# rusty-fast-solvers/rusty-compression

Measured on AMD Instinct MI355X. Metric: GB/s + compressions/sec, 8192x8192 f64 rank-128 rSVD+ID, higher is better.
Workload: dtype f64

## Files before the change

rusty_compression_amd/csrc/kernels_tsqr.hip:

```cpp
#include "rc_common.hpp"
#include "rc_device.hpp"

namespace rc {

static __host__ __device__ inline int64_t cdiv(int64_t a, int64_t b) { return (a + b - 1) / b; }

template <typename T> struct TNum;
template <> struct TNum<double> {
    static __device__ inline double tol3z() { return 1.0536712127723509e-08; }
    static __device__ inline double tiny() { return 1e-300; }
};
template <> struct TNum<float> {
    static __device__ inline float tol3z() { return 2.44140625e-04f; }
    static __device__ inline float tiny() { return 1e-30f; }
};

template <typename T>
__device__ inline T wave_sum64(T v) {
#pragma unroll
    for (int off = 32; off > 0; off >>= 1) v += __shfl_xor(v, off, 64);
    return v;
}
template <typename T>
__device__ inline T row_sum16(T v) {
#pragma unroll
    for (int off = 8; off > 0; off >>= 1) v += __shfl_xor(v, off, 64);
    return v;
}

template <typename T, int NT>
__global__ __launch_bounds__(1024) void k_chol_inv(Mat<T> g, Mat<T> r_out, Mat<T> rinv_out, int check_identity, T ident_tol, T skip_tol, int *flag) {
    extern __shared__ __attribute__((aligned(16))) char smem_raw[];
    const int n = (int)g.rows;
    const int ld = n | 1;
    T *A = reinterpret_cast<T *>(smem_raw);
    T *svec = A + (size_t)n * ld;
    T *rowbuf = svec + n;
    T *red = rowbuf + 2 * n;
    const int tid = threadIdx.x, lane = tid & 63, wv = tid >> 6;
    const int ti = tid >> 5, tc = tid & 31;

    T reg[NT][NT];
    T dev = 0;
#pragma unroll
    for (int a = 0; a < NT; ++a)
#pragma unroll
        for (int b = 0; b < NT; ++b) {
            const int i = ti + 32 * a, c = tc + 32 * b;
            T v = 0;
            if (i < n && c < n) {
                v = g.at(i, c);
                dev = max(dev, fabs(v - ((i == c) ? (T)1 : (T)0)));
            }
            reg[a][b] = v;
// ... 74 lines not shown
                }
            } else if (i > j && i < n) {
                const T w = rb[i] * invd;
#pragma unroll
                for (int b = a; b < NT; ++b) reg[a][b] -= w * cv[b];
            }
            if (i <= j) {
                const T xj = cb[i];
                const T w = xj * invd;
#pragma unroll
                for (int b = a; b < NT; ++b) {
                    xr[a][b] -= w * cv[b];
                    if (b == ja && tc == jt) xr[a][b] = xj * invr;
                }
            }
        }
    }
#pragma unroll
    for (int a = 0; a < NT; ++a)
#pragma unroll
        for (int b = 0; b < NT; ++b) {
            const int i = ti + 32 * a, c = tc + 32 * b;
            if (i < n && c < n) {
                r_out.at(i, c) = (b >= a && c >= i) ? reg[a][b] : (T)0;
                rinv_out.at(i, c) = (b >= a && c >= i) ? xr[a][b] : (T)0;
            }
        }
}

template <typename T>
static size_t chol_lds(int64_t n) { return ((size_t)n * (n | 1) + 3 * (size_t)n + 16) * sizeof(T); }

template <typename T, int NT>
static void chol_inv_launch(rc_context *c, Mat<T> g, Mat<T> r, Mat<T> rinv, bool check_identity, T ident_tol, T skip_tol, int *flag) {
    auto kern = k_chol_inv<T, NT>;
    static bool attr_set[64] = {};
    if (!attr_set[c->device & 63]) {
        RC_HIP(hipFuncSetAttribute(reinterpret_cast<const void *>(kern), hipFuncAttributeMaxDynamicSharedMemorySize, 160 * 1024 - 1024));
        attr_set[c->device & 63] = true;
    }
    hipLaunchKernelGGL(kern, dim3(1), dim3(1024), chol_lds<T>(g.rows), c->stream, g, r, rinv, check_identity ? 1 : 0, ident_tol, skip_tol, flag);
}
template <typename T>
static void chol_inv(rc_context *c, Mat<T> g, Mat<T> r, Mat<T> rinv, bool check_identity, T ident_tol, T skip_tol, int *flag) {
    const int64_t n = g.rows;
    RC_REQUIRE(n <= 224 && chol_lds<T>(n) <= 160 * 1024 - 1024, RC_INVALID_ARGUMENT, "chol_inv: n = %lld does not fit LDS", (long long)n);
    ProfScope ps(c, "op:chol_inv n=%lld", (long long)n);
    if (n <= 64) chol_inv_launch<T, 2>(c, g, r, rinv, check_identity, ident_tol, skip_tol, flag);
    else if (n <= 160) chol_inv_launch<T, 5>(c, g, r, rinv, check_identity, ident_tol, skip_tol, flag);
    else chol_inv_launch<T, 7>(c, g, r, rinv, check_identity, ident_tol, skip_tol, flag);
}

template <typename T>
bool tsqr_supported(int64_t m, int64_t n) {
    const size_t small_lds = ((size_t)n * (n | 1) + 4 * (size_t)n) * sizeof(T) + (size_t)n * sizeof(int) + 256;
    return n >= 2 && m >= 4 * n && m >= 1024 && small_lds <= 160 * 1024 - 2048;
}

template <typename T>
void tsqr_cholqr2_factored(rc_context *c, Mat<T> y, Mat<T> q1, Mat<T> r2i, Mat<T> r, int *flag) {
    const int64_t m = y.rows, n = y.cols;
    ProfScope ps(c, "op:cholqr2 %lldx%lld", (long long)m, (long long)n);
    ArenaMark mark(c);
    Mat<T> g = rowmajor(c->alloc<T>((size_t)n * even_ld(n)), n, n, even_ld(n));
    Mat<T> r1 = rowmajor(c->alloc<T>((size_t)n * even_ld(n)), n, n, even_ld(n)), r1i = rowmajor(c->alloc<T>((size_t)n * even_ld(n)), n, n, even_ld(n));
    Mat<T> r2 = rowmajor(c->alloc<T>((size_t)n * even_ld(n)), n, n, even_ld(n));
    gemm<T>(c, 1, y.t(), y, 0, g);
    chol_inv<T>(c, g, r1, r1i, false, 0, 0, flag);
    gemm<T>(c, 1, y, r1i, 0, q1);
    gemm<T>(c, 1, q1.t(), q1, 0, g);
    static const int skip_ok = [] { const char *e = getenv("RC_CHOLQR_SKIP"); return e ? atoi(e) : 1; }();
    const T skip_tol = skip_ok ? (sizeof(T) == 8 ? (T)2.5e-14 : (T)1e-6) : (T)-1;
    chol_inv<T>(c, g, r2, r2i, true, (T)1e-2, skip_tol, flag);
    gemm<T>(c, 1, r2, r1, 0, r);
}

template <typename T>
void tsqr_cholqr2(rc_context *c, Mat<T> y, Mat<T> q, Mat<T> r, int *flag) {
    const int64_t m = y.rows, n = y.cols;
    ArenaMark mark(c);
    Mat<T> q1 = rowmajor(c->alloc<T>((size_t)m * even_ld(n)), m, n, even_ld(n));
    Mat<T> r2i = rowmajor(c->alloc<T>((size_t)n * even_ld(n)), n, n, even_ld(n));
    tsqr_cholqr2_factored<T>(c, y, q1, r2i, r, flag);
    gemm<T>(c, 1, q1, r2i, 0, q);
}

template <typename T>
__device__ inline T safe_hypot(T a, T b) {
    a = fabs(a); b = fabs(b);
    const T w = max(a, b), z = min(a, b);
    if (z == (T)0) return w;
    const T q = z * fast_rcp(w);
    const T e = (T)1 + q * q;
    return w * (e * fast_rsqrt(e));
}
template <typename T>
__device__ inline T fast_sqrt_pos(T x) { return x > (T)0 ? x * fast_rsqrt(x) : (T)0; }

template <typename T, int NEJ, int LPP>
__device__ __forceinline__ void qrcp_small_apply(T *A, int ld, int n, int j, int grp, int ll, int ngrp, const int *jp, T *vn1, T *vn2, T tj, int pivot, bool safe) {
    const T *vcol = A + jp[j] * ld;
    T v[NEJ];
#pragma unroll
    for (int e = 0; e < NEJ; ++e) {
        int i = j + ll + LPP * e;
        v[e] = (i < n) ? ((i == j) ? (T)1 : vcol[i]) : (T)0;
    }
    for (int p = j + 1 + grp; p < n; p += ngrp) {
        T *xcol = A + jp[p] * ld;
        T x[NEJ];
        T dot = 0;
        if (safe) {
#pragma unroll
            for (int e = 0; e < NEJ; ++e) {
                x[e] = xcol[j + ll + LPP * e];
                dot = fma(v[e], x[e], dot);
            }
        } else {
#pragma unroll
            for (int e = 0; e < NEJ; ++e) {
                int i = j + ll + LPP * e;
                x[e] = (i < n) ? xcol[i] : (T)0;
                dot = fma(v[e], x[e], dot);
            }
        }
        if (tj != (T)0) {
            dot = group_sum_dpp<LPP>(dot);
            const T f = tj * dot;
#pragma unroll
            for (int e = 0; e < NEJ; ++e) {
                int i = j + ll + LPP * e;
                if (i < n) { x[e] -= f * v[e]; xcol[i] = x[e]; }
            }
        }
        if (pivot) {
            const T xj = xcol[j];
            const T vn = vn1[p];
            if (vn != (T)0) {
                T t = fabs(xj) * fast_rcp(vn);
                T temp = (T)1 - t * t;
                temp = temp > (T)0 ? temp : (T)0;
                T rr = vn * fast_rcp(vn2[p]);
                T temp2 = temp * rr * rr;
                if (temp2 <= TNum<T>::tol3z()) {
                    T ss = 0;
#pragma unroll
                    for (int e = 0; e < NEJ; ++e) {
                        int i = j + ll + LPP * e;
                        if (i > j && i < n) ss += x[e] * x[e];
                    }
                    ss = group_sum_dpp<LPP>(ss);
                    if (ll == 0) { T nn = (j < n - 1) ? fast_sqrt_pos(ss) : (T)0; vn1[p] = nn; vn2[p] = nn; }
                } else if (ll == 0) {
                    vn1[p] = vn * fast_sqrt_pos(temp);
                }
            }
        }
    }
}

template <typename T, int NE, int LPP, int E0>
__device__ __forceinline__ void qrcp_small_reflect(T (&x)[NE], const T *vcol, T tj, int j, int n, int ll) {
    T v[NE];
    T dot = 0;
#pragma unroll
    for (int e = E0; e < NE; ++e) {
        int i = ll + LPP * e;
        v[e] = 0;
        if (i < n && i >= j) { v[e] = (i == j) ? (T)1 : vcol[i]; dot = fma(v[e], x[e], dot); }
    }
    dot = group_sum_dpp<LPP>(dot);
    const T f = tj * dot;
#pragma unroll
    for (int e = E0; e < NE; ++e) x[e] -= f * v[e];
}

template <typename T, int NE, int NTHR>
__global__ __launch_bounds__(NTHR) void k_qrcp_small(Mat<T> rin, int kmax, int pivot, int64_t *jpvt_out, Mat<T> rout, Mat<T> q2) {
    constexpr int LPP = 8;
    constexpr int NGRP = NTHR / LPP;
    extern __shared__ __attribute__((aligned(16))) char smem_raw[];
    const int n = (int)rin.rows;
    const int ld = n | 1;
    T *A = reinterpret_cast<T *>(smem_raw);
    T *vn1 = A + (size_t)n * ld;
    T *vn2 = vn1 + n;
    T *tau = vn2 + n;
    int *jp = reinterpret_cast<int *>(tau + n);
    const int tid = threadIdx.x, lane = tid & 63;
    const int ll = tid % LPP, grp = tid / LPP;
    const bool safe = LPP * NE <= 3 * n;

    for (int e = tid; e < n * n; e += NTHR) {
        int i = e % n, cc = e / n;
        A[cc * ld + i] = rin.at(i, cc);
    }
    __syncthreads();
    for (int p = grp; p < n; p += NGRP) {
        T acc = 0;
        for (int i = ll; i < n; i += LPP) { T v = A[p * ld + i]; acc += v * v; }
        acc = group_sum_dpp<LPP>(acc);
        if (ll == 0) { T nr = sqrt(acc); vn1[p] = nr; vn2[p] = nr; jp[p] = p; tau[p] = (T)0; }
    }
    __syncthreads();

    for (int j = 0; j < kmax; ++j) {
        if (tid < 64) {
            if (pivot) {
                T best = (T)-1;
                int bi = 0x7fffffff;
                for (int p = j + lane; p < n; p += 64) {
                    T v = fabs(vn1[p]);
                    if (v > best) { best = v; bi = p; }
                }
                const T mx = wave_max_dpp(best);
                const int pv = wave_min_dpp(best == mx ? bi : 0x7fffffff);
                const int pvt = (pv >= j && pv < n) ? pv : j;
                if (lane == 0 && pvt != j) {
                    int t = jp[pvt]; jp[pvt] = jp[j]; jp[j] = t;
                    vn1[pvt] = vn1[j];
                    vn2[pvt] = vn2[j];
                }
                __builtin_amdgcn_fence(__ATOMIC_ACQ_REL, "wavefront");
            }
            T *col = A + jp[j] * ld;
            const T alpha = col[j];
            T acc = 0;
            for (int i = j + 1 + lane; i < n; i += 64) { T v = col[i]; acc += v * v; }
            acc = wave_sum_dpp(acc);
            const T xnorm = fast_sqrt_pos(acc);
            if (xnorm == (T)0) {
                if (lane == 0) tau[j] = 0;
            } else {
                const T beta = -copysign(safe_hypot(alpha, xnorm), alpha);
                const T scal = fast_rcp(alpha - beta);
                for (int i = j + 1 + lane; i < n; i += 64) col[i] *= scal;
                if (lane == 0) { tau[j] = (beta - alpha) * fast_rcp(beta); col[j] = beta; }
            }
        }
        __syncthreads();
        {
            const int rem = n - j;
            const T tj = tau[j];
            if (NE > 12 && rem > 8 * 12) qrcp_small_apply<T, NE, LPP>(A, ld, n, j, grp, ll, NGRP, jp, vn1, vn2, tj, pivot, safe);
            else if (NE > 8 && rem > 8 * 8) qrcp_small_apply<T, (NE > 12 ? 12 : NE), LPP>(A, ld, n, j, grp, ll, NGRP, jp, vn1, vn2, tj, pivot, safe);
            else if (NE > 4 && rem > 8 * 4) qrcp_small_apply<T, (NE > 8 ? 8 : NE), LPP>(A, ld, n, j, grp, ll, NGRP, jp, vn1, vn2, tj, pivot, safe);
            else qrcp_small_apply<T, (NE > 4 ? 4 : NE), LPP>(A, ld, n, j, grp, ll, NGRP, jp, vn1, vn2, tj, pivot, safe);
        }
        __syncthreads();
    }

    for (int p = tid; p < n; p += NTHR) jpvt_out[p] = jp[p];
    if (!rout.empty()) {
        const int64_t total = rout.rows * rout.cols;
        for (int64_t e = tid; e < total; e += NTHR) {
            int i = (int)(e / rout.cols), p = (int)(e % rout.cols);
            rout.at(i, p) = (i <= p) ? A[jp[p] * ld + i] : (T)0;
        }
    }
    if (!q2.empty()) {
        for (int cq = grp; cq < (int)q2.cols; cq += NGRP) {
            T x[NE];
#pragma unroll
            for (int e = 0; e < NE; ++e) x[e] = (ll + LPP * e == cq) ? (T)1 : (T)0;
            for (int j = (cq < kmax - 1 ? cq : kmax - 1); j >= 0; --j) {
                const T tj = tau[j];
                if (tj == (T)0) continue;
                const T *vcol = A + jp[j] * ld;
                const int e0 = j / LPP;
                if (NE > 12 && e0 >= 12) qrcp_small_reflect<T, NE, LPP, (NE > 12 ? 12 : 0)>(x, vcol, tj, j, n, ll);
                else if (NE > 8 && e0 >= 8) qrcp_small_reflect<T, NE, LPP, (NE > 8 ? 8 : 0)>(x, vcol, tj, j, n, ll);
                else if (NE > 4 && e0 >= 4) qrcp_small_reflect<T, NE, LPP, (NE > 4 ? 4 : 0)>(x, vcol, tj, j, n, ll);
                else qrcp_small_reflect<T, NE, LPP, 0>(x, vcol, tj, j, n, ll);
            }
#pragma unroll
            for (int e = 0; e < NE; ++e) {
                int i = ll + LPP * e;
                if (i < n) q2.at(i, cq) = x[e];
            }
        }
    }
}

template <typename T>
void qrcp_small(rc_context *c, Mat<T> rin, int64_t kmax, bool pivot, int64_t *jpvt, Mat<T> rout, Mat<T> q2) {
    const int64_t n = rin.rows;
    RC_REQUIRE(rin.rows == rin.cols, RC_INVALID_ARGUMENT, "qrcp_small: square input required");
    const size_t lds = ((size_t)n * (n | 1) + 3 * (size_t)n) * sizeof(T) + (size_t)n * sizeof(int) + 64;
    RC_REQUIRE(lds <= 160 * 1024 - 1024 && n <= 208, RC_INVALID_ARGUMENT, "qrcp_small: n = %lld does not fit LDS", (long long)n);
    ProfScope ps(c, "op:qrcp_small n=%lld k=%lld", (long long)n, (long long)kmax);
#define RC_QS(NE, NT_)                                                                                                 \
    do {                                                                                                               \
        auto kern = k_qrcp_small<T, NE, NT_>;                                                                          \
        static bool attr_set[64] = {};                                                                                 \
        if (!attr_set[c->device & 63]) {                                                                               \
            RC_HIP(hipFuncSetAttribute(reinterpret_cast<const void *>(kern), hipFuncAttributeMaxDynamicSharedMemorySize, 160 * 1024 - 1024)); \
            attr_set[c->device & 63] = true;                                                                           \
        }                                                                                                              \
        hipLaunchKernelGGL(kern, dim3(1), dim3(NT_), lds, c->stream, rin, (int)kmax, pivot ? 1 : 0, jpvt, rout, q2);   \
    } while (0)
    static const int wide = [] { const char *e = getenv("RC_QRCP_SMALL_1024"); return e ? atoi(e) : 1; }();
    if (n <= 64) RC_QS(8, 512);
    else if (n <= 144 && wide) RC_QS(18, 1024);
    else if (n <= 144) RC_QS(18, 512);
    else RC_QS(26, 512);
#undef RC_QS
}

template <typename T>
__global__ __launch_bounds__(1024) void k_householder_signs(Mat<T> q, T *d) {
    extern __shared__ __attribute__((aligned(16))) char smem_raw[];
    const int k = (int)q.cols;
    const int ld = k | 1;
    T *W = reinterpret_cast<T *>(smem_raw);
    const int tid = threadIdx.x;
    for (int e = tid; e < k * k; e += 1024) {
        int i = e % k, cc = e / k;
        W[i * ld + cc] = q.at(i, cc);
    }
    __syncthreads();
    const int ti = tid >> 5, tc = tid & 31;
    for (int j = 0; j < k; ++j) {
        const T s = W[j * ld + j];
        const T dj = (s > (T)0) ? (T)-1 : (T)1;
        const T u = (T)1 + fabs(s);
        if (tid == 0) d[j] = dj;
        const T inv = -dj / u;
        for (int i = j + 1 + ti; i < k; i += 32) {
            const T li = W[i * ld + j] * inv;
            for (int cc = j + 1 + tc; cc < k; cc += 32) W[i * ld + cc] -= li * W[j * ld + cc];
        }
        __syncthreads();
    }
}
template <typename T>
__global__ __launch_bounds__(256) void k_scale_cols_rows(Mat<T> q, Mat<T> r, const T *d) {
    const int64_t tq = q.rows * q.cols, tr = r.rows * r.cols;
    for (int64_t e = blockIdx.x * (int64_t)blockDim.x + threadIdx.x; e < tq + tr; e += (int64_t)gridDim.x * blockDim.x) {
        if (e < tq) {
            int64_t j = e / q.rows, i = e - j * q.rows;
            if (d[j] < (T)0) q.at(i, j) = -q.at(i, j);
        } else {
            int64_t f = e - tq;
            int64_t i = f / r.cols, p = f - i * r.cols;
            if (d[i] < (T)0) r.at(i, p) = -r.at(i, p);
        }
    }
}

template <typename T>
static void householder_signs(rc_context *c, Mat<T> top, T *d) {
    const int64_t k = top.cols;
    const size_t lds = (size_t)k * (k | 1) * sizeof(T);
    RC_REQUIRE(top.rows >= k && lds <= 160 * 1024 - 1024, RC_INVALID_ARGUMENT, "sign fix: k = %lld does not fit LDS", (long long)k);
    auto kern = k_householder_signs<T>;
    static bool attr_set[64] = {};
    if (!attr_set[c->device & 63]) {
        RC_HIP(hipFuncSetAttribute(reinterpret_cast<const void *>(kern), hipFuncAttributeMaxDynamicSharedMemorySize, 160 * 1024 - 1024));
        attr_set[c->device & 63] = true;
    }
    hipLaunchKernelGGL(kern, dim3(1), dim3(1024), lds, c->stream, top, d);
}
template <typename T>
static void scale_cols_rows(rc_context *c, Mat<T> q, Mat<T> r, const T *d) {
    const int64_t total = q.rows * q.cols + r.rows * r.cols;
    hipLaunchKernelGGL(k_scale_cols_rows<T>, dim3((unsigned)std::min<int64_t>(cdiv(total, 256), 4096)), dim3(256), 0, c->stream, q, r, d);
}

template <typename T>
void householder_sign_fix(rc_context *c, Mat<T> q, Mat<T> r) {
    const int64_t k = q.cols;
    if (k == 0) return;
    RC_REQUIRE(q.rows >= k, RC_INVALID_ARGUMENT, "sign fix: q must be tall");
    ProfScope ps(c, "op:householder_sign_fix k=%lld", (long long)k);
    ArenaMark mark(c);
    T *d = c->alloc<T>((size_t)k);
    householder_signs<T>(c, q, d);
    scale_cols_rows<T>(c, q, r, d);
}

template <typename T>
void qrcp_tall_fast(rc_context *c, Mat<T> y, int64_t k, bool pivot, Mat<T> q, Mat<T> r, int64_t *ind, int *flag) {
    const int64_t m = y.rows, n = y.cols;
    ProfScope ps(c, "op:qrcp_tall_fast %lldx%lld k=%lld pivot=%d", (long long)m, (long long)n, (long long)k, pivot ? 1 : 0);
    ArenaMark mark(c);
    static const int fold = [] { const char *e = getenv("RC_TSQR_FOLD"); return e ? atoi(e) : 1; }();
    Mat<T> q1 = rowmajor(c->alloc<T>((size_t)m * even_ld(n)), m, n, even_ld(n));
    Mat<T> r1 = colmajor(c->alloc<T>((size_t)n * even_ld(n)), n, n, even_ld(n));
    Mat<T> r2i = rowmajor(c->alloc<T>((size_t)n * even_ld(n)), n, n, even_ld(n));
    if (fold) tsqr_cholqr2_factored<T>(c, y, q1, r2i, r1, flag);
    else tsqr_cholqr2<T>(c, y, q1, r1, flag);
    Mat<T> q2 = colmajor(c->alloc<T>((size_t)even_ld(n) * k), n, k, even_ld(n));
    Mat<T> rr = r.empty() ? rowmajor(c->alloc<T>((size_t)k * even_ld(n)), k, n, even_ld(n)) : r;
    qrcp_small<T>(c, r1, k, pivot, ind, rr, q2);
    Mat<T> qq = q.empty() ? rowmajor(c->alloc<T>((size_t)m * even_ld(k)), m, k, even_ld(k)) : q;
    if (!fold) {
        gemm<T>(c, 1, q1, q2, 0, qq);
        householder_sign_fix<T>(c, qq, rr);
        return;
    }
    Mat<T> w = colmajor(c->alloc<T>((size_t)even_ld(n) * k), n, k, even_ld(n));
    Mat<T> top = colmajor(c->alloc<T>((size_t)even_ld(k) * k), k, k, even_ld(k));
    T *d = c->alloc<T>((size_t)k);
    gemm<T>(c, 1, r2i, q2, 0, w);
    gemm<T>(c, 1, q1.sub(0, k, 0, n), w, 0, top);
    householder_signs<T>(c, top, d);
    scale_cols_rows<T>(c, w, rr, d);
    gemm<T>(c, 1, q1, w, 0, qq);
}

#define RC_INST(T)                                                                                               \
    template bool tsqr_supported<T>(int64_t, int64_t);                                                           \
    template void tsqr_cholqr2<T>(rc_context *, Mat<T>, Mat<T>, Mat<T>, int *);                                  \
    template void tsqr_cholqr2_factored<T>(rc_context *, Mat<T>, Mat<T>, Mat<T>, Mat<T>, int *);                 \
    template void qrcp_small<T>(rc_context *, Mat<T>, int64_t, bool, int64_t *, Mat<T>, Mat<T>);                 \
    template void householder_sign_fix<T>(rc_context *, Mat<T>, Mat<T>);                                         \
    template void qrcp_tall_fast<T>(rc_context *, Mat<T>, int64_t, bool, Mat<T>, Mat<T>, int64_t *, int *);
RC_INST(double)
RC_INST(float)
#undef RC_INST

}
```

rusty_compression_amd/csrc/rc_api.hip:

```cpp
#include "rc_common.hpp"

#include <unistd.h>

#include <atomic>
#include <chrono>

#include <algorithm>
#include <cmath>

using namespace rc;

static constexpr size_t kAlign = 256;

void rc_context::retire_arena() {
    if (arena) {
        if (live_graphs > 0) retired.push_back(arena);
        else (void)hipFree(arena);
    }
    arena = nullptr;
    arena_size = 0;
}

void rc_context::swap_arena() {
    std::swap(arena, aux_arena.base);
// ... 201 lines not shown
    RC_HIP(hipMemcpyAsync(c->pinned, dev, bytes, hipMemcpyDeviceToHost, c->stream));
    RC_HIP(hipStreamSynchronize(c->stream));
    std::memcpy(host, c->pinned, bytes);
}

template <typename T>
Mat<T> tmp_colmajor(rc_context *c, int64_t rows, int64_t cols) {
    int64_t ld = even_ld(std::max<int64_t>(rows, 1));
    return colmajor(c->alloc<T>((size_t)ld * std::max<int64_t>(cols, 1)), rows, cols, ld);
}
template <typename T>
Mat<T> tmp_rowmajor(rc_context *c, int64_t rows, int64_t cols) {
    int64_t ld = even_ld(std::max<int64_t>(cols, 1));
    return rowmajor(c->alloc<T>((size_t)ld * std::max<int64_t>(rows, 1)), rows, cols, ld);
}

void check_view(const rc_matrix &m, const char *name, bool allow_null = false) {
    RC_REQUIRE(m.rows >= 0 && m.cols >= 0, RC_INVALID_ARGUMENT, "%s: negative extent", name);
    if (!allow_null) RC_REQUIRE(m.data != nullptr || m.rows == 0 || m.cols == 0, RC_INVALID_ARGUMENT, "%s: null data", name);
}


__global__ void k_or_flag(int *dst, const int *src) {
    if (threadIdx.x == 0 && blockIdx.x == 0 && *src) atomicOr(dst, *src);
}
__global__ void k_set_word(int *dst, int v) {
    if (threadIdx.x == 0 && blockIdx.x == 0) *dst = v;
}

static int debug_memset_path() {
    static const int v = [] { const char *e = getenv("RC_DEBUG_MEMSET_PATH"); return e ? atoi(e) : 0; }();
    return v;
}

template <typename F>
bool run_certified(rc_context *c, F &&fast) {
    int *flag = c->alloc<int>(1);
    if (debug_memset_path() & 1) RC_HIP(hipMemsetAsync(flag, 0, sizeof(int), c->stream));
    else hipLaunchKernelGGL(k_set_word, dim3(1), dim3(64), 0, c->stream, flag, 0);
    fast(flag);
    if (c->capturing) {
        hipLaunchKernelGGL(k_or_flag, dim3(1), dim3(64), 0, c->stream, c->health_word(), flag);
        return true;
    }
    int h = 0;
    read_back(c, flag, &h, 1);
    return h == 0;
}

template <typename T>
void qrcp_core(rc_context *c, Mat<T> w, int64_t k, bool pivot, Mat<T> q, Mat<T> r, int64_t *ind, bool keep_w = false) {
    const int64_t n = w.cols;
    ArenaMark mark(c);
    if (c->opt_tsqr && k >= 1 && tsqr_supported<T>(w.rows, n)) {
        if (run_certified(c, [&](int *flag) { qrcp_tall_fast<T>(c, w, k, pivot, q, r, ind, flag); })) return;
    }
    static const int direct_ok = [] { const char *e = getenv("RC_QRCP_KEEP_DIRECT"); return e ? atoi(e) : 1; }();
    if (keep_w && !(direct_ok && c->opt_wide_coop && pivot && k >= 1 && wide_coop_supported<T>(w.rows, n, c->device))) {
        Mat<T> cp = tmp_colmajor<T>(c, w.rows, n);
        copy_mat(c, w, cp);
        w = cp;
        keep_w = false;
    }
    if (c->opt_wide_coop && pivot && k >= 1 && wide_coop_supported<T>(w.rows, n, c->device)) {
        T *tau = c->alloc<T>((size_t)k);
        Mat<T> wf = tmp_colmajor<T>(c, w.rows, n);
        if (run_certified(c, [&](int *flag) { geqp3_wide_coop<T>(c, w, wf, k, ind, tau, flag); })) {
            if (!r.empty()) extract_r(c, wf, ind, r);
            if (!q.empty()) {
                if (q.rs == 1 && q.cs >= q.rows) {
                    form_q(c, wf, ind, tau, k, q);
                } else {
                    Mat<T> qw = tmp_colmajor<T>(c, w.rows, q.cols);
                    form_q(c, wf, ind, tau, k, qw);
                    copy_mat(c, qw, q);
                }
            }
            return;
        }
    }
    if (keep_w) {
        Mat<T> cp = tmp_colmajor<T>(c, w.rows, n);
        copy_mat(c, w, cp);
        w = cp;
    }
    if (c->opt_wide_lazy && pivot && k >= 1 && wide_lazy_supported<T>(w.rows, n)) {
        geqp3_wide_lazy<T>(c, w, k, ind, q, r);
        return;
    }
    T *tau = c->alloc<T>((size_t)std::max<int64_t>(k, 1));
    if (c->opt_blocked && pivot && !c->capturing && geqp3_blocked_supported<T>(w.rows, n, k)) {
        const bool direct = !q.empty() && q.rs == 1 && q.cs >= q.rows;
        Mat<T> qw = q.empty() ? Mat<T>() : (direct ? q : tmp_colmajor<T>(c, w.rows, q.cols));
        geqp3_blocked<T>(c, w, k, ind, tau, qw);
        if (!r.empty()) extract_r(c, w, ind, r);
        if (!q.empty() && !direct) copy_mat(c, qw, q);
        return;
    }
    T *vn = c->alloc<T>((size_t)std::max<int64_t>(2 * n, 1));
    geqp3_inplace(c, w, k, pivot, ind, tau, vn);
    if (!r.empty()) extract_r(c, w, ind, r);
    if (!q.empty()) {
        if (q.rs == 1 && q.cs >= q.rows) {
            form_q(c, w, ind, tau, k, q);
        } else {
            Mat<T> qw = tmp_colmajor<T>(c, w.rows, q.cols);
            form_q(c, w, ind, tau, k, qw);
            copy_mat(c, qw, q);
// ... 1126 lines not shown
```

rusty_compression_amd/csrc/rc_common.hpp:

```cpp
#pragma once

#include <hip/hip_runtime.h>

#include <cstdarg>
#include <cstdint>
#include <cstdio>
#include <cstring>
#include <map>
#include <string>
#include <vector>

#include "../../include/rusty_compression_amd.h"

namespace rc {

template <typename T>
struct Mat {
    T *p = nullptr;
    int64_t rows = 0, cols = 0, rs = 0, cs = 0;

    __host__ __device__ Mat() {}
    __host__ __device__ Mat(T *p_, int64_t r, int64_t c, int64_t rs_, int64_t cs_) : p(p_), rows(r), cols(c), rs(rs_), cs(cs_) {}
    __host__ __device__ inline T &at(int64_t i, int64_t j) const { return p[i * rs + j * cs]; }
    __host__ __device__ Mat<T> sub(int64_t r0, int64_t nr, int64_t c0, int64_t nc) const {
// ... 134 lines not shown
void philox_words(rc_context *c, uint32_t *out, int64_t n, uint64_t seed, uint64_t word_offset);
template <typename T> void copy_mat(rc_context *c, Mat<T> src, Mat<T> dst);
template <typename T> void fill_identity(rc_context *c, Mat<T> dst);
template <typename T> void fill_zero(rc_context *c, Mat<T> dst);
template <typename T> void scale_rows(rc_context *c, const T *s, Mat<T> src, Mat<T> dst);
template <typename T> void gather_cols(rc_context *c, Mat<T> src, const int64_t *idx, Mat<T> dst);
template <typename T> void column_id_from_qrcp(rc_context *c, Mat<T> a, Mat<T> w, int64_t k, const int64_t *jpvt, Mat<T> cm, Mat<T> z);
template <typename T> void id_z_from_r(rc_context *c, Mat<T> r, int64_t k, const int64_t *ind, Mat<T> z);
template <typename T> void batched_column_id(rc_context *c, Mat<T> a, int64_t abs, int32_t count, int64_t k, double tol, Mat<T> cm, int64_t cbs, Mat<T> z,
                                             int64_t zbs, int64_t *col_ind, int64_t *ranks);
template <typename T> void batched_two_sided_id(rc_context *c, Mat<T> a, int64_t abs, int32_t count, int64_t k, double tol, Mat<T> cm, int64_t cbs, Mat<T> x,
                                                int64_t xbs, Mat<T> z, int64_t zbs, int64_t *row_ind, int64_t *col_ind, int64_t *ranks);
void invert_perm(rc_context *c, const int64_t *perm, int64_t n, int64_t *inv);
void fill_words(rc_context *c, void *p, size_t bytes, unsigned v);
void iota_i64(rc_context *c, int64_t *p, int64_t n);
template <typename T> void col_sumsq(rc_context *c, Mat<T> a, T *out);
template <typename T> void max_sqrt(rc_context *c, const T *v, int64_t n, T *out);
template <typename T> void fro_diff(rc_context *c, Mat<T> a, Mat<T> b, T *out2);
template <typename T> void adaptive_residual_update(rc_context *c, Mat<T> y, Mat<T> corr);

template <typename T> void gemm(rc_context *c, T alpha, Mat<T> a, Mat<T> b, T beta, Mat<T> cmat);
template <typename T> void complete_left_basis(rc_context *c, Mat<T> uc, const T *s);

template <typename T> void geqp3_inplace(rc_context *c, Mat<T> w, int64_t kmax, bool pivot, int64_t *jpvt, T *tau, T *vn);
template <typename T> bool geqp3_blocked_supported(int64_t m, int64_t n, int64_t kmax);
template <typename T> void geqp3_blocked(rc_context *c, Mat<T> w, int64_t kmax, int64_t *jpvt, T *tau, Mat<T> q_out, Mat<T> restore_from = Mat<T>());
template <typename T> struct BlockedQrcpJob;
template <typename T> BlockedQrcpJob<T> *qrb_begin(rc_context *c, Mat<T> w, int64_t kmax, int64_t *jpvt, T *tau);
template <typename T> void qrb_issue(BlockedQrcpJob<T> *job);
template <typename T> bool qrb_finish(BlockedQrcpJob<T> *job);
template <typename T> void qrb_form_q(BlockedQrcpJob<T> *job, Mat<T> q);
template <typename T> void qrb_end(BlockedQrcpJob<T> *job);
struct QrbState;
template <typename T> bool qrb_optimistic_possible(BlockedQrcpJob<T> *job);
template <typename T> bool qrb_issue_all_optimistic(BlockedQrcpJob<T> *job);
template <typename T> bool qrb_verify_optimistic(BlockedQrcpJob<T> *job);
template <typename T> bool qrb_verify_optimistic(const QrbState *host_log, const std::vector<int> &nbp_log, bool broken);
template <typename T> void qrb_optimistic_log(BlockedQrcpJob<T> *job, const QrbState **log, std::vector<int> *nbp_log, bool *broken);
template <typename T> void qrb_keep_t(BlockedQrcpJob<T> *job, bool keep);
template <typename T> bool wide_lazy_supported(int64_t m, int64_t n);
template <typename T> void geqp3_wide_lazy(rc_context *c, Mat<T> b, int64_t kmax, int64_t *jpvt, Mat<T> q, Mat<T> r);
template <typename T> bool wide_coop_supported(int64_t m, int64_t n, int device);
template <typename T> void geqp3_wide_coop(rc_context *c, Mat<T> w, Mat<T> wf, int64_t kmax, int64_t *jpvt, T *tau, int *flag);
void coop_prepare(int device);
unsigned *coop_semaphore_of(int device);
unsigned coop_budget_units(int device);
void coop_gate_launch(rc_context *c, unsigned need, unsigned *sync, unsigned long long *hdr, int hdr_words, const int *proceed = nullptr);
template <typename T> void extract_r(rc_context *c, Mat<T> w, const int64_t *jpvt, Mat<T> r);
template <typename T> void form_q(rc_context *c, Mat<T> w, const int64_t *jpvt, const T *tau, int64_t k, Mat<T> qw);
template <typename T> void trsm_upper(rc_context *c, Mat<T> t, Mat<T> b);
template <typename T> bool tsqr_supported(int64_t m, int64_t n);
template <typename T> void tsqr_cholqr2(rc_context *c, Mat<T> y, Mat<T> q, Mat<T> r, int *flag);
template <typename T> void tsqr_cholqr2_factored(rc_context *c, Mat<T> y, Mat<T> q1, Mat<T> r2i, Mat<T> r, int *flag);
template <typename T> void qrcp_small(rc_context *c, Mat<T> rin, int64_t kmax, bool pivot, int64_t *jpvt, Mat<T> rout, Mat<T> q2);
template <typename T> void householder_sign_fix(rc_context *c, Mat<T> q, Mat<T> r);
template <typename T> void qrcp_tall_fast(rc_context *c, Mat<T> y, int64_t k, bool pivot, Mat<T> q, Mat<T> r, int64_t *ind, int *flag);
template <typename T> void jacobi_svd(rc_context *c, Mat<T> g, Mat<T> vwork, Mat<T> uc, T *s, Mat<T> vc);

}
```

Baseline: 600.6.

## Replace CholQR2+small Householder QRCP with pivoted Cholesky on Gram matrix

The tall pivoted QR path changes. It used to run CholQR2 on the full n-column matrix, then a shared-memory Householder QRCP on R, then fold and sign-fix. Now a single-block pivoted Cholesky kernel works directly on the Gram matrix Y^T Y and produces the pivots, R rows and the inverse factor W1 for only k columns. One CholQR refinement pass on the resulting m×k Q1 follows. This removes the n×n Cholesky/inverse, a full-width Y·R1^-1 GEMM and the separate QRCP kernel, at the cost of pivoting on a squared-condition Gram matrix. That may trip the certification flag more often and fall back to the slow path. The fast path is now restricted to pivot=true, and the supported n shrinks for f64.

```diff
diff --git a/rusty_compression_amd/csrc/kernels_tsqr.hip b/rusty_compression_amd/csrc/kernels_tsqr.hip
--- a/rusty_compression_amd/csrc/kernels_tsqr.hip
+++ b/rusty_compression_amd/csrc/kernels_tsqr.hip
@@ -1,5 +1,7 @@
 #include "rc_common.hpp"
 #include "rc_device.hpp"
+
+#include <limits>
 
 namespace rc {
 
@@ -180,9 +182,23 @@
 }
 
 template <typename T>
+static T cholqr_skip_tol() {
+    static const int skip_ok = [] { const char *e = getenv("RC_CHOLQR_SKIP"); return e ? atoi(e) : 1; }();
+    return skip_ok ? (sizeof(T) == 8 ? (T)2.5e-14 : (T)1e-6) : (T)-1;
+}
+
+template <typename T>
+static size_t pchol_lds(int64_t n, int64_t kmax) { return ((size_t)kmax * n + 2 * (size_t)kmax) * sizeof(T) + 2 * (size_t)n * sizeof(int); }
+template <typename T>
+static constexpr int64_t pchol_nmax() { return sizeof(T) == 8 ? 160 : 224; }
+template <typename T>
+static size_t signs_lds(int64_t k) { return (size_t)k * (k | 1) * sizeof(T); }
+
+template <typename T>
 bool tsqr_supported(int64_t m, int64_t n) {
-    const size_t small_lds = ((size_t)n * (n | 1) + 4 * (size_t)n) * sizeof(T) + (size_t)n * sizeof(int) + 256;
-    return n >= 2 && m >= 4 * n && m >= 1024 && small_lds <= 160 * 1024 - 2048;
+    constexpr size_t lds_max = 160 * 1024 - 1024;
+    return n >= 2 && m >= 4 * n && m >= 1024 && n <= pchol_nmax<T>() && pchol_lds<T>(n, n) <= lds_max && chol_lds<T>(n) <= lds_max &&
+           signs_lds<T>(n) <= lds_max;
 }
 
 template <typename T>
@@ -197,9 +213,7 @@
     chol_inv<T>(c, g, r1, r1i, false, 0, 0, flag);
     gemm<T>(c, 1, y, r1i, 0, q1);
     gemm<T>(c, 1, q1.t(), q1, 0, g);
-    static const int skip_ok = [] { const char *e = getenv("RC_CHOLQR_SKIP"); return e ? atoi(e) : 1; }();
-    const T skip_tol = skip_ok ? (sizeof(T) == 8 ? (T)2.5e-14 : (T)1e-6) : (T)-1;
-    chol_inv<T>(c, g, r2, r2i, true, (T)1e-2, skip_tol, flag);
+    chol_inv<T>(c, g, r2, r2i, true, (T)1e-2, cholqr_skip_tol<T>(), flag);
     gemm<T>(c, 1, r2, r1, 0, r);
 }
 
@@ -213,226 +227,161 @@
     gemm<T>(c, 1, q1, r2i, 0, q);
 }
 
-template <typename T>
-__device__ inline T safe_hypot(T a, T b) {
-    a = fabs(a); b = fabs(b);
-    const T w = max(a, b), z = min(a, b);
-    if (z == (T)0) return w;
-    const T q = z * fast_rcp(w);
-    const T e = (T)1 + q * q;
-    return w * (e * fast_rsqrt(e));
-}
-template <typename T>
-__device__ inline T fast_sqrt_pos(T x) { return x > (T)0 ? x * fast_rsqrt(x) : (T)0; }
-
-template <typename T, int NEJ, int LPP>
-__device__ __forceinline__ void qrcp_small_apply(T *A, int ld, int n, int j, int grp, int ll, int ngrp, const int *jp, T *vn1, T *vn2, T tj, int pivot, bool safe) {
-    const T *vcol = A + jp[j] * ld;
-    T v[NEJ];
-#pragma unroll
-    for (int e = 0; e < NEJ; ++e) {
-        int i = j + ll + LPP * e;
-        v[e] = (i < n) ? ((i == j) ? (T)1 : vcol[i]) : (T)0;
-    }
-    for (int p = j + 1 + grp; p < n; p += ngrp) {
-        T *xcol = A + jp[p] * ld;
-        T x[NEJ];
-        T dot = 0;
-        if (safe) {
-#pragma unroll
-            for (int e = 0; e < NEJ; ++e) {
-                x[e] = xcol[j + ll + LPP * e];
-                dot = fma(v[e], x[e], dot);
-            }
-        } else {
-#pragma unroll
-            for (int e = 0; e < NEJ; ++e) {
-                int i = j + ll + LPP * e;
-                x[e] = (i < n) ? xcol[i] : (T)0;
-                dot = fma(v[e], x[e], dot);
-            }
-        }
-        if (tj != (T)0) {
-            dot = group_sum_dpp<LPP>(dot);
-            const T f = tj * dot;
-#pragma unroll
-            for (int e = 0; e < NEJ; ++e) {
-                int i = j + ll + LPP * e;
-                if (i < n) { x[e] -= f * v[e]; xcol[i] = x[e]; }
-            }
-        }
-        if (pivot) {
-            const T xj = xcol[j];
-            const T vn = vn1[p];
-            if (vn != (T)0) {
-                T t = fabs(xj) * fast_rcp(vn);
-                T temp = (T)1 - t * t;
-                temp = temp > (T)0 ? temp : (T)0;
-                T rr = vn * fast_rcp(vn2[p]);
-                T temp2 = temp * rr * rr;
-                if (temp2 <= TNum<T>::tol3z()) {
-                    T ss = 0;
-#pragma unroll
-                    for (int e = 0; e < NEJ; ++e) {
-                        int i = j + ll + LPP * e;
-                        if (i > j && i < n) ss += x[e] * x[e];
+template <typename T, int NT>
+__global__ __launch_bounds__(1024) void k_pchol_inv(Mat<T> g, int kmax, int64_t *jpvt_out, Mat<T> rout, Mat<T> w1, int *flag) {
+    extern __shared__ __attribute__((aligned(16))) char smem_raw[];
+    const int n = (int)g.rows;
+    T *rows = reinterpret_cast<T *>(smem_raw);
+    T *rdg = rows + (size_t)kmax * n;
+    T *rsc = rdg + kmax;
+    int *jp = reinterpret_cast<int *>(rsc + kmax);
+    int *cpos = jp + n;
+    const int tid = threadIdx.x, lane = tid & 63, wv = tid >> 6;
+    const int ti = tid >> 5, tc = tid & 31;
+
+    T m[NT][NT];
+    T d[NT];
+    int pos[NT];
+    unsigned rdone = 0;
+    T dmax = 0;
+#pragma unroll
+    for (int a = 0; a < NT; ++a) {
+        const int i = ti + 32 * a;
+        if (i >= n) rdone |= 1u << a;
+#pragma unroll
+        for (int b = 0; b < NT; ++b) {
+            const int c = tc + 32 * b;
+            m[a][b] = (i < n && c < n) ? g.at(i, c) : (T)0;
+        }
+    }
+#pragma unroll
+    for (int b = 0; b < NT; ++b) {
+        const int c = tc + 32 * b;
+        const T v = (c < n) ? g.at(c, c) : (T)0;
+        d[b] = v > (T)0 ? v : (T)0;
+        pos[b] = c;
+        dmax = max(dmax, d[b]);
+    }
+    const T negl = std::numeric_limits<T>::epsilon() * wave_max_dpp(dmax);
+
+    for (int j = 0; j < kmax; ++j) {
+        T best = (T)-1;
+        int key = 0x7fffffff;
+#pragma unroll
+        for (int b = 0; b < NT; ++b) {
+            const int c = tc + 32 * b;
+            const int kk = (pos[b] << 8) | c;
+            if (c < n && pos[b] >= j && (d[b] > best || (d[b] == best && kk < key))) { best = d[b]; key = kk; }
+        }
+        const T mx = wave_max_dpp(best);
+        const int pk = wave_min_dpp(best == mx ? key : 0x7fffffff);
+        const int pvt = pk >> 8, p = pk & 255;
+        const int pa = p >> 5, pt = p & 31;
+        T *rb = rows + (size_t)j * n;
+        if (ti == pt) {
+#pragma unroll
+            for (int a = 0; a < NT; ++a)
+                if (a == pa) {
+#pragma unroll
+                    for (int b = 0; b < NT; ++b) {
+                        const int c = tc + 32 * b;
+                        if (c < n) rb[c] = (c == p) ? (T)1 : m[a][b];
                     }
-                    ss = group_sum_dpp<LPP>(ss);
-                    if (ll == 0) { T nn = (j < n - 1) ? fast_sqrt_pos(ss) : (T)0; vn1[p] = nn; vn2[p] = nn; }
-                } else if (ll == 0) {
-                    vn1[p] = vn * fast_sqrt_pos(temp);
-                }
-            }
-        }
-    }
-}
-
-template <typename T, int NE, int LPP, int E0>
-__device__ __forceinline__ void qrcp_small_reflect(T (&x)[NE], const T *vcol, T tj, int j, int n, int ll) {
-    T v[NE];
-    T dot = 0;
-#pragma unroll
-    for (int e = E0; e < NE; ++e) {
-        int i = ll + LPP * e;
-        v[e] = 0;
-        if (i < n && i >= j) { v[e] = (i == j) ? (T)1 : vcol[i]; dot = fma(v[e], x[e], dot); }
-    }
-    dot = group_sum_dpp<LPP>(dot);
-    const T f = tj * dot;
-#pragma unroll
-    for (int e = E0; e < NE; ++e) x[e] -= f * v[e];
-}
-
-template <typename T, int NE, int NTHR>
-__global__ __launch_bounds__(NTHR) void k_qrcp_small(Mat<T> rin, int kmax, int pivot, int64_t *jpvt_out, Mat<T> rout, Mat<T> q2) {
-    constexpr int LPP = 8;
-    constexpr int NGRP = NTHR / LPP;
-    extern __shared__ __attribute__((aligned(16))) char smem_raw[];
-    const int n = (int)rin.rows;
-    const int ld = n | 1;
-    T *A = reinterpret_cast<T *>(smem_raw);
-    T *vn1 = A + (size_t)n * ld;
-    T *vn2 = vn1 + n;
-    T *tau = vn2 + n;
-    int *jp = reinterpret_cast<int *>(tau + n);
-    const int tid = threadIdx.x, lane = tid & 63;
-    const int ll = tid % LPP, grp = tid / LPP;
-    const bool safe = LPP * NE <= 3 * n;
-
-    for (int e = tid; e < n * n; e += NTHR) {
-        int i = e % n, cc = e / n;
-        A[cc * ld + i] = rin.at(i, cc);
+                }
+        }
+        __syncthreads();
+        T dp = mx;
+        if (!(dp > negl) || !(dp <= std::numeric_limits<T>::max())) {
+            if (tid == 0) atomicOr(flag, 1);
+            if (!(dp > (T)0)) dp = TNum<T>::tiny();
+        }
+        const T invr = fast_rsqrt(dp), invd = invr * invr;
+        T cv[NT];
+#pragma unroll
+        for (int b = 0; b < NT; ++b) { const int c = tc + 32 * b; cv[b] = (c < n) ? rb[c] : (T)0; }
+        if (tid == 0) { rdg[j] = dp * invr; rsc[j] = invr; }
+#pragma unroll
+        for (int a = 0; a < NT; ++a) {
+            const int i = ti + 32 * a;
+            if (i == p) {
+#pragma unroll
+                for (int b = 0; b < NT; ++b) {
+                    const int c = tc + 32 * b;
+                    m[a][b] = (c == p) ? invr : (pos[b] < j ? m[a][b] * invr : (T)0);
+                }
+            } else if (!((rdone >> a) & 1u)) {
+                const T w = rb[i] * invd;
+#pragma unroll
+                for (int b = 0; b < NT; ++b) {
+                    const int c = tc + 32 * b;
+                    m[a][b] = ((c == p) ? (T)0 : m[a][b]) - w * cv[b];
+                }
+            }
+        }
+        if (ti == pt) rdone |= 1u << pa;
+#pragma unroll
+        for (int b = 0; b < NT; ++b) {
+            const int c = tc + 32 * b;
+            if (c == p) {
+                pos[b] = j;
+            } else if (pos[b] >= j) {
+                const T t = cv[b] * invr;
+                const T v = d[b] - t * t;
+                d[b] = v > (T)0 ? v : (T)0;
+                if (pos[b] == j) pos[b] = pvt;
+            }
+        }
+    }
+
+    if (wv == 0 && lane < 32) {
+#pragma unroll
+        for (int b = 0; b < NT; ++b) {
+            const int c = tc + 32 * b;
+            if (c < n) { jp[pos[b]] = c; cpos[c] = pos[b]; }
+        }
     }
     __syncthreads();
-    for (int p = grp; p < n; p += NGRP) {
-        T acc = 0;
-        for (int i = ll; i < n; i += LPP) { T v = A[p * ld + i]; acc += v * v; }
-        acc = group_sum_dpp<LPP>(acc);
-        if (ll == 0) { T nr = sqrt(acc); vn1[p] = nr; vn2[p] = nr; jp[p] = p; tau[p] = (T)0; }
-    }
-    __syncthreads();
-
-    for (int j = 0; j < kmax; ++j) {
-        if (tid < 64) {
-            if (pivot) {
-                T best = (T)-1;
-                int bi = 0x7fffffff;
-                for (int p = j + lane; p < n; p += 64) {
-                    T v = fabs(vn1[p]);
-                    if (v > best) { best = v; bi = p; }
-                }
-                const T mx = wave_max_dpp(best);
-                const int pv = wave_min_dpp(best == mx ? bi : 0x7fffffff);
-                const int pvt = (pv >= j && pv < n) ? pv : j;
-                if (lane == 0 && pvt != j) {
-                    int t = jp[pvt]; jp[pvt] = jp[j]; jp[j] = t;
-                    vn1[pvt] = vn1[j];
-                    vn2[pvt] = vn2[j];
-                }
-                __builtin_amdgcn_fence(__ATOMIC_ACQ_REL, "wavefront");
-            }
-            T *col = A + jp[j] * ld;
-            const T alpha = col[j];
-            T acc = 0;
-            for (int i = j + 1 + lane; i < n; i += 64) { T v = col[i]; acc += v * v; }
-            acc = wave_sum_dpp(acc);
-            const T xnorm = fast_sqrt_pos(acc);
-            if (xnorm == (T)0) {
-                if (lane == 0) tau[j] = 0;
-            } else {
-                const T beta = -copysign(safe_hypot(alpha, xnorm), alpha);
-                const T scal = fast_rcp(alpha - beta);
-                for (int i = j + 1 + lane; i < n; i += 64) col[i] *= scal;
-                if (lane == 0) { tau[j] = (beta - alpha) * fast_rcp(beta); col[j] = beta; }
-            }
-        }
-        __syncthreads();
-        {
-            const int rem = n - j;
-            const T tj = tau[j];
-            if (NE > 12 && rem > 8 * 12) qrcp_small_apply<T, NE, LPP>(A, ld, n, j, grp, ll, NGRP, jp, vn1, vn2, tj, pivot, safe);
-            else if (NE > 8 && rem > 8 * 8) qrcp_small_apply<T, (NE > 12 ? 12 : NE), LPP>(A, ld, n, j, grp, ll, NGRP, jp, vn1, vn2, tj, pivot, safe);
-            else if (NE > 4 && rem > 8 * 4) qrcp_small_apply<T, (NE > 8 ? 8 : NE), LPP>(A, ld, n, j, grp, ll, NGRP, jp, vn1, vn2, tj, pivot, safe);
-            else qrcp_small_apply<T, (NE > 4 ? 4 : NE), LPP>(A, ld, n, j, grp, ll, NGRP, jp, vn1, vn2, tj, pivot, safe);
-        }
-        __syncthreads();
-    }
-
-    for (int p = tid; p < n; p += NTHR) jpvt_out[p] = jp[p];
+    for (int p = tid; p < n; p += 1024) jpvt_out[p] = jp[p];
+#pragma unroll
+    for (int a = 0; a < NT; ++a) {
+        const int i = ti + 32 * a;
+        const int pj = (i < n) ? cpos[i] : kmax;
+        if (pj < kmax) {
+#pragma unroll
+            for (int b = 0; b < NT; ++b) {
+                const int c = tc + 32 * b;
+                if (c < n) w1.at(c, pj) = m[a][b];
+            }
+        }
+    }
     if (!rout.empty()) {
-        const int64_t total = rout.rows * rout.cols;
-        for (int64_t e = tid; e < total; e += NTHR) {
-            int i = (int)(e / rout.cols), p = (int)(e % rout.cols);
-            rout.at(i, p) = (i <= p) ? A[jp[p] * ld + i] : (T)0;
-        }
-    }
-    if (!q2.empty()) {
-        for (int cq = grp; cq < (int)q2.cols; cq += NGRP) {
-            T x[NE];
-#pragma unroll
-            for (int e = 0; e < NE; ++e) x[e] = (ll + LPP * e == cq) ? (T)1 : (T)0;
-            for (int j = (cq < kmax - 1 ? cq : kmax - 1); j >= 0; --j) {
-                const T tj = tau[j];
-                if (tj == (T)0) continue;
-                const T *vcol = A + jp[j] * ld;
-                const int e0 = j / LPP;
-                if (NE > 12 && e0 >= 12) qrcp_small_reflect<T, NE, LPP, (NE > 12 ? 12 : 0)>(x, vcol, tj, j, n, ll);
-                else if (NE > 8 && e0 >= 8) qrcp_small_reflect<T, NE, LPP, (NE > 8 ? 8 : 0)>(x, vcol, tj, j, n, ll);
-                else if (NE > 4 && e0 >= 4) qrcp_small_reflect<T, NE, LPP, (NE > 4 ? 4 : 0)>(x, vcol, tj, j, n, ll);
-                else qrcp_small_reflect<T, NE, LPP, 0>(x, vcol, tj, j, n, ll);
-            }
-#pragma unroll
-            for (int e = 0; e < NE; ++e) {
-                int i = ll + LPP * e;
-                if (i < n) q2.at(i, cq) = x[e];
-            }
-        }
-    }
-}
-
-template <typename T>
-void qrcp_small(rc_context *c, Mat<T> rin, int64_t kmax, bool pivot, int64_t *jpvt, Mat<T> rout, Mat<T> q2) {
-    const int64_t n = rin.rows;
-    RC_REQUIRE(rin.rows == rin.cols, RC_INVALID_ARGUMENT, "qrcp_small: square input required");
-    const size_t lds = ((size_t)n * (n | 1) + 3 * (size_t)n) * sizeof(T) + (size_t)n * sizeof(int) + 64;
-    RC_REQUIRE(lds <= 160 * 1024 - 1024 && n <= 208, RC_INVALID_ARGUMENT, "qrcp_small: n = %lld does not fit LDS", (long long)n);
-    ProfScope ps(c, "op:qrcp_small n=%lld k=%lld", (long long)n, (long long)kmax);
-#define RC_QS(NE, NT_)                                                                                                 \
-    do {                                                                                                               \
-        auto kern = k_qrcp_small<T, NE, NT_>;                                                                          \
-        static bool attr_set[64] = {};                                                                                 \
-        if (!attr_set[c->device & 63]) {                                                                               \
-            RC_HIP(hipFuncSetAttribute(reinterpret_cast<const void *>(kern), hipFuncAttributeMaxDynamicSharedMemorySize, 160 * 1024 - 1024)); \
-            attr_set[c->device & 63] = true;                                                                           \
-        }                                                                                                              \
-        hipLaunchKernelGGL(kern, dim3(1), dim3(NT_), lds, c->stream, rin, (int)kmax, pivot ? 1 : 0, jpvt, rout, q2);   \
-    } while (0)
-    static const int wide = [] { const char *e = getenv("RC_QRCP_SMALL_1024"); return e ? atoi(e) : 1; }();
-    if (n <= 64) RC_QS(8, 512);
-    else if (n <= 144 && wide) RC_QS(18, 1024);
-    else if (n <= 144) RC_QS(18, 512);
-    else RC_QS(26, 512);
-#undef RC_QS
+        for (int e = tid; e < kmax * n; e += 1024) {
+            const int i = e / n, pp = e - i * n;
+            rout.at(i, pp) = (pp > i) ? rows[(size_t)i * n + jp[pp]] * rsc[i] : (pp == i ? rdg[i] : (T)0);
+        }
+    }
+}
+
+template <typename T, int NT>
+static void pchol_inv_launch(rc_context *c, Mat<T> g, int kmax, int64_t *jpvt, Mat<T> rout, Mat<T> w1, int *flag) {
+    auto kern = k_pchol_inv<T, NT>;
+    static bool attr_set[64] = {};
+    if (!attr_set[c->device & 63]) {
+        RC_HIP(hipFuncSetAttribute(reinterpret_cast<const void *>(kern), hipFuncAttributeMaxDynamicSharedMemorySize, 160 * 1024 - 1024));
+        attr_set[c->device & 63] = true;
+    }
+    hipLaunchKernelGGL(kern, dim3(1), dim3(1024), pchol_lds<T>(g.rows, kmax), c->stream, g, kmax, jpvt, rout, w1, flag);
+}
+template <typename T>
+static void pchol_inv(rc_context *c, Mat<T> g, int64_t kmax, int64_t *jpvt, Mat<T> rout, Mat<T> w1, int *flag) {
+    const int64_t n = g.rows;
+    RC_REQUIRE(g.cols == n && n <= pchol_nmax<T>() && kmax >= 1 && kmax <= n && pchol_lds<T>(n, kmax) <= 160 * 1024 - 1024, RC_INVALID_ARGUMENT,
+               "pchol_inv: n = %lld, k = %lld not supported", (long long)n, (long long)kmax);
+    RC_REQUIRE(w1.rows == n && w1.cols == kmax && (rout.empty() || (rout.rows == kmax && rout.cols == n)), RC_INVALID_ARGUMENT, "pchol_inv: output shapes");
+    ProfScope ps(c, "op:pchol_inv n=%lld k=%lld", (long long)n, (long long)kmax);
+    if (n <= 64) pchol_inv_launch<T, 2>(c, g, (int)kmax, jpvt, rout, w1, flag);
+    else if (n <= 160) pchol_inv_launch<T, 5>(c, g, (int)kmax, jpvt, rout, w1, flag);
+    else if constexpr (sizeof(T) == 4) pchol_inv_launch<T, 7>(c, g, (int)kmax, jpvt, rout, w1, flag);
 }
 
 template <typename T>
@@ -479,7 +428,7 @@
 template <typename T>
 static void householder_signs(rc_context *c, Mat<T> top, T *d) {
     const int64_t k = top.cols;
-    const size_t lds = (size_t)k * (k | 1) * sizeof(T);
+    const size_t lds = signs_lds<T>(k);
     RC_REQUIRE(top.rows >= k && lds <= 160 * 1024 - 1024, RC_INVALID_ARGUMENT, "sign fix: k = %lld does not fit LDS", (long long)k);
     auto kern = k_householder_signs<T>;
     static bool attr_set[64] = {};
@@ -496,54 +445,36 @@
 }
 
 template <typename T>
-void householder_sign_fix(rc_context *c, Mat<T> q, Mat<T> r) {
-    const int64_t k = q.cols;
-    if (k == 0) return;
-    RC_REQUIRE(q.rows >= k, RC_INVALID_ARGUMENT, "sign fix: q must be tall");
-    ProfScope ps(c, "op:householder_sign_fix k=%lld", (long long)k);
+void qrcp_tall_fast(rc_context *c, Mat<T> y, int64_t k, Mat<T> q, Mat<T> r, int64_t *ind, int *flag) {
+    const int64_t m = y.rows, n = y.cols;
+    ProfScope ps(c, "op:qrcp_tall_fast %lldx%lld k=%lld", (long long)m, (long long)n, (long long)k);
     ArenaMark mark(c);
-    T *d = c->alloc<T>((size_t)k);
-    householder_signs<T>(c, q, d);
-    scale_cols_rows<T>(c, q, r, d);
-}
-
-template <typename T>
-void qrcp_tall_fast(rc_context *c, Mat<T> y, int64_t k, bool pivot, Mat<T> q, Mat<T> r, int64_t *ind, int *flag) {
-    const int64_t m = y.rows, n = y.cols;
-    ProfScope ps(c, "op:qrcp_tall_fast %lldx%lld k=%lld pivot=%d", (long long)m, (long long)n, (long long)k, pivot ? 1 : 0);
-    ArenaMark mark(c);
-    static const int fold = [] { const char *e = getenv("RC_TSQR_FOLD"); return e ? atoi(e) : 1; }();
-    Mat<T> q1 = rowmajor(c->alloc<T>((size_t)m * even_ld(n)), m, n, even_ld(n));
-    Mat<T> r1 = colmajor(c->alloc<T>((size_t)n * even_ld(n)), n, n, even_ld(n));
-    Mat<T> r2i = rowmajor(c->alloc<T>((size_t)n * even_ld(n)), n, n, even_ld(n));
-    if (fold) tsqr_cholqr2_factored<T>(c, y, q1, r2i, r1, flag);
-    else tsqr_cholqr2<T>(c, y, q1, r1, flag);
-    Mat<T> q2 = colmajor(c->alloc<T>((size_t)even_ld(n) * k), n, k, even_ld(n));
-    Mat<T> rr = r.empty() ? rowmajor(c->alloc<T>((size_t)k * even_ld(n)), k, n, even_ld(n)) : r;
-    qrcp_small<T>(c, r1, k, pivot, ind, rr, q2);
-    Mat<T> qq = q.empty() ? rowmajor(c->alloc<T>((size_t)m * even_ld(k)), m, k, even_ld(k)) : q;
-    if (!fold) {
-        gemm<T>(c, 1, q1, q2, 0, qq);
-        householder_sign_fix<T>(c, qq, rr);
-        return;
-    }
-    Mat<T> w = colmajor(c->alloc<T>((size_t)even_ld(n) * k), n, k, even_ld(n));
+    Mat<T> g = rowmajor(c->alloc<T>((size_t)n * even_ld(n)), n, n, even_ld(n));
+    Mat<T> w1 = rowmajor(c->alloc<T>((size_t)n * even_ld(k)), n, k, even_ld(k));
+    Mat<T> rt;
+    if (!r.empty()) rt = rowmajor(c->alloc<T>((size_t)k * even_ld(n)), k, n, even_ld(n));
+    Mat<T> q1 = rowmajor(c->alloc<T>((size_t)m * even_ld(k)), m, k, even_ld(k));
+    gemm<T>(c, 1, y.t(), y, 0, g);
+    pchol_inv<T>(c, g, k, ind, rt, w1, flag);
+    gemm<T>(c, 1, y, w1, 0, q1);
+    Mat<T> g2 = rowmajor(c->alloc<T>((size_t)k * even_ld(k)), k, k, even_ld(k));
+    Mat<T> r2 = rowmajor(c->alloc<T>((size_t)k * even_ld(k)), k, k, even_ld(k)), r2i = rowmajor(c->alloc<T>((size_t)k * even_ld(k)), k, k, even_ld(k));
+    gemm<T>(c, 1, q1.t(), q1, 0, g2);
+    chol_inv<T>(c, g2, r2, r2i, true, (T)1e-2, cholqr_skip_tol<T>(), flag);
+    if (!r.empty()) gemm<T>(c, 1, r2, rt, 0, r);
     Mat<T> top = colmajor(c->alloc<T>((size_t)even_ld(k) * k), k, k, even_ld(k));
     T *d = c->alloc<T>((size_t)k);
-    gemm<T>(c, 1, r2i, q2, 0, w);
-    gemm<T>(c, 1, q1.sub(0, k, 0, n), w, 0, top);
+    gemm<T>(c, 1, q1.sub(0, k, 0, k), r2i, 0, top);
     householder_signs<T>(c, top, d);
-    scale_cols_rows<T>(c, w, rr, d);
-    gemm<T>(c, 1, q1, w, 0, qq);
+    scale_cols_rows<T>(c, r2i, r, d);
+    if (!q.empty()) gemm<T>(c, 1, q1, r2i, 0, q);
 }
 
 #define RC_INST(T)                                                                                               \
     template bool tsqr_supported<T>(int64_t, int64_t);                                                           \
     template void tsqr_cholqr2<T>(rc_context *, Mat<T>, Mat<T>, Mat<T>, int *);                                  \
     template void tsqr_cholqr2_factored<T>(rc_context *, Mat<T>, Mat<T>, Mat<T>, Mat<T>, int *);                 \
-    template void qrcp_small<T>(rc_context *, Mat<T>, int64_t, bool, int64_t *, Mat<T>, Mat<T>);                 \
-    template void householder_sign_fix<T>(rc_context *, Mat<T>, Mat<T>);                                         \
-    template void qrcp_tall_fast<T>(rc_context *, Mat<T>, int64_t, bool, Mat<T>, Mat<T>, int64_t *, int *);
+    template void qrcp_tall_fast<T>(rc_context *, Mat<T>, int64_t, Mat<T>, Mat<T>, int64_t *, int *);
 RC_INST(double)
 RC_INST(float)
 #undef RC_INST
diff --git a/rusty_compression_amd/csrc/rc_api.hip b/rusty_compression_amd/csrc/rc_api.hip
--- a/rusty_compression_amd/csrc/rc_api.hip
+++ b/rusty_compression_amd/csrc/rc_api.hip
@@ -277,8 +277,8 @@
 void qrcp_core(rc_context *c, Mat<T> w, int64_t k, bool pivot, Mat<T> q, Mat<T> r, int64_t *ind, bool keep_w = false) {
     const int64_t n = w.cols;
     ArenaMark mark(c);
-    if (c->opt_tsqr && k >= 1 && tsqr_supported<T>(w.rows, n)) {
-        if (run_certified(c, [&](int *flag) { qrcp_tall_fast<T>(c, w, k, pivot, q, r, ind, flag); })) return;
+    if (c->opt_tsqr && pivot && k >= 1 && tsqr_supported<T>(w.rows, n)) {
+        if (run_certified(c, [&](int *flag) { qrcp_tall_fast<T>(c, w, k, q, r, ind, flag); })) return;
     }
     static const int direct_ok = [] { const char *e = getenv("RC_QRCP_KEEP_DIRECT"); return e ? atoi(e) : 1; }();
     if (keep_w && !(direct_ok && c->opt_wide_coop && pivot && k >= 1 && wide_coop_supported<T>(w.rows, n, c->device))) {
diff --git a/rusty_compression_amd/csrc/rc_common.hpp b/rusty_compression_amd/csrc/rc_common.hpp
--- a/rusty_compression_amd/csrc/rc_common.hpp
+++ b/rusty_compression_amd/csrc/rc_common.hpp
@@ -210,9 +210,7 @@
 template <typename T> bool tsqr_supported(int64_t m, int64_t n);
 template <typename T> void tsqr_cholqr2(rc_context *c, Mat<T> y, Mat<T> q, Mat<T> r, int *flag);
 template <typename T> void tsqr_cholqr2_factored(rc_context *c, Mat<T> y, Mat<T> q1, Mat<T> r2i, Mat<T> r, int *flag);
-template <typename T> void qrcp_small(rc_context *c, Mat<T> rin, int64_t kmax, bool pivot, int64_t *jpvt, Mat<T> rout, Mat<T> q2);
-template <typename T> void householder_sign_fix(rc_context *c, Mat<T> q, Mat<T> r);
-template <typename T> void qrcp_tall_fast(rc_context *c, Mat<T> y, int64_t k, bool pivot, Mat<T> q, Mat<T> r, int64_t *ind, int *flag);
+template <typename T> void qrcp_tall_fast(rc_context *c, Mat<T> y, int64_t k, Mat<T> q, Mat<T> r, int64_t *ind, int *flag);
 template <typename T> void jacobi_svd(rc_context *c, Mat<T> g, Mat<T> vwork, Mat<T> uc, T *s, Mat<T> vc);
 
 }
```

Result: faster. 622.0 (median of 6 runs) (+3.6%).
